# victorvg17/Towards-Interpretable-Reinforcement-Learning-Using-Attention-Augmented-Agents-Replication

Hardware: AMD Instinct MI355X
Metric: learner frames/sec (fwd+bwd, T=20 unroll) at 1/2/4/8 MI355X + % roofline (higher is better)
Workload: dtype fp32; 1 GPU; C2 (BASELINE.json configs[1]): B=32 per GPU x T=20 unroll, 84x84, 4 heads, fp32; global_batch=32, seq_len=20, frame=84x84, heads=4, parallelism=dp1

## Files before the change

### towards-interpretable-reinforcement-learning-using-attention-augmented-agents-replication_amd/csrc/gemm.h

```cpp
#pragma once
#include <type_traits>
#include "common.h"

namespace aaa {

template <typename T, int R, int BK, bool KC>
struct Tile {
  static constexpr int PAD = (!KC && sizeof(T) == 2) ? 32 : 16 / (int)sizeof(T);
  static constexpr int LD = KC ? (BK + PAD) : (R + PAD);
  static constexpr int ELEMS = (KC ? R : BK) * LD;
  __device__ static __forceinline__ int off(int r, int k) { return KC ? r * LD + k : k * LD + r; }
};

template <typename G, typename T, int R, int BK, int NT>
struct LdRows {
  static constexpr bool KC = true;
  static constexpr int VG = 16 / (int)sizeof(G);
  static constexpr int CPR = BK / VG;
  static constexpr int NCH = R * CPR;
  static constexpr int PER = (NCH + NT - 1) / NT;
  struct Params { const G* src; int ld; int nrows; };
  const G* rowp[PER];
  int kc[PER], lr[PER];
  bool ok[PER], act[PER];
// ... 196 lines not shown
  using Regs = u32x4[PER];
  __device__ __forceinline__ LdIm2colT(const Params& p, int row0) : g(p.g), src(p.src) {
#pragma unroll
    for (int c = 0; c < PER; ++c) {
      int ch = threadIdx.x + c * NT;
      act[c] = ch < NCH;
      kr[c] = ch / CPK;
      rc[c] = (ch % CPK) * VG;
      constexpr int NE = VEC ? 1 : 4;
#pragma unroll
      for (int e = 0; e < NE; ++e) {
        int kp = row0 + rc[c] + e;
        rok[c][e] = act[c] && kp < p.nrows;
        int kq = rok[c][e] ? kp : 0;
        int tap = (int)g.dCin.div(kq);
        ci[c][e] = kq - tap * g.Cin;
        ky[c][e] = (int)g.dKW.div(tap);
        kx[c][e] = tap - ky[c][e] * g.KW;
      }
    }
  }
  __device__ __forceinline__ void fetch(int k0, int kend, Regs& buf) const {
    const int hw = g.Hout * g.Wout;
#pragma unroll
    for (int c = 0; c < PER; ++c) {
      u32x4 v = u32x4{0, 0, 0, 0};
      int m = k0 + kr[c];
      if (act[c] && m < kend) {
        int f = (int)g.dHW.div(m), pix = m - f * hw;
        int oy = (int)g.dWout.div(pix), ox = pix - oy * g.Wout;
        const G* fb = src + (size_t)f * g.Hin * g.Win * g.cs + g.coff;
        if constexpr (VEC) {
          int iy, ix;
          if (rok[c][0] && conv_src(g, oy, ox, ky[c][0], kx[c][0], iy, ix))
            v = *reinterpret_cast<const u32x4*>(fb + (size_t)(iy * g.Win + ix) * g.cs + ci[c][0]);
        } else {
          static_assert(sizeof(G) == 4, "scalar im2col path expects fp32 global data");
          float tmp[4] = {0.f, 0.f, 0.f, 0.f};
#pragma unroll
          for (int e = 0; e < 4; ++e) {
            int iy, ix;
            if (rok[c][e] && conv_src(g, oy, ox, ky[c][e], kx[c][e], iy, ix))
              tmp[e] = (float)fb[(size_t)(iy * g.Win + ix) * g.cs + ci[c][e]];
          }
          v = __builtin_bit_cast(u32x4, tmp);
        }
      }
      buf[c] = v;
    }
  }
  __device__ __forceinline__ void commit(T* lds, const Regs& buf) const {
#pragma unroll
    for (int c = 0; c < PER; ++c)
      if (NCH % NT == 0 || act[c]) lds_store_chunk<G, T>(lds + Tile<T, R, BK, false>::off(rc[c], kr[c]), buf[c]);
  }
};

template <typename TL>
__device__ __forceinline__ void frag_f32(const float* t, int r, int k, float (&a)[8]) {
  if constexpr (TL::KC_) {
    const f32x4* p = reinterpret_cast<const f32x4*>(t + r * TL::LD + k);
    f32x4 x = p[0], y = p[1];
    a[0] = x[0]; a[1] = x[1]; a[2] = x[2]; a[3] = x[3];
    a[4] = y[0]; a[5] = y[1]; a[6] = y[2]; a[7] = y[3];
  } else {
#pragma unroll
    for (int kk = 0; kk < 8; ++kk) a[kk] = t[(k + kk) * TL::LD + r];
  }
}

typedef short s16x4 __attribute__((ext_vector_type(4)));
typedef __attribute__((address_space(3))) s16x4 lds_s16x4;

template <typename TL>
__device__ __forceinline__ bf16x8 frag_bf16(const __bf16* t, int r, int k) {
  if constexpr (TL::KC_) {
    return *reinterpret_cast<const bf16x8*>(t + r * TL::LD + k);
  } else {
    const int li = (int)(threadIdx.x & 15), q = li >> 2, p = li & 3;
    const __bf16* a0 = t + (k + q) * TL::LD + (r - li) + 4 * p;
    const s16x4 lo = __builtin_amdgcn_ds_read_tr16_b64_v4i16((lds_s16x4*)(const_cast<__bf16*>(a0)));
    const s16x4 hi = __builtin_amdgcn_ds_read_tr16_b64_v4i16((lds_s16x4*)(const_cast<__bf16*>(a0 + 4 * TL::LD)));
    typedef short s16x8 __attribute__((ext_vector_type(8)));
    const s16x8 v = {lo[0], lo[1], lo[2], lo[3], hi[0], hi[1], hi[2], hi[3]};
    return __builtin_bit_cast(bf16x8, v);
  }
}

struct TileMap {
  int remap;
  FastDiv ny, nxy;
};
__device__ __forceinline__ void tile_of(const TileMap& m, int& ti, int& tj, int& tz) {
  if (!m.remap) { ti = blockIdx.y; tj = blockIdx.x; tz = blockIdx.z; return; }
  const int ny = (int)m.ny.d, nxy = (int)m.nxy.d, n = nxy * gridDim.z;
  const int b = (blockIdx.z * ny + blockIdx.y) * gridDim.x + blockIdx.x;
  const int q = n >> 3, r = n & 7, x = b & 7;
  const int t = (x < r ? x * (q + 1) : r * (q + 1) + (x - r) * q) + (b >> 3);
  tz = (int)m.nxy.div((uint32_t)t);
  const int u = t - tz * nxy;
  tj = (int)m.ny.div((uint32_t)u);
  ti = u - tj * ny;
}
inline int xcd_remap_enabled() {
#ifdef AAA_ABLATION
  const char* e = getenv("AAA_XCD_REMAP");
  return e ? atoi(e) != 0 : 1;
#else
  return 1;
#endif
}
inline TileMap tile_map(dim3 grid) {
  TileMap m;
  m.remap = xcd_remap_enabled();
  m.ny = FastDiv(grid.y);
  m.nxy = FastDiv(grid.x * grid.y);
  return m;
}

template <typename T, int R, int BK, bool KC>
struct TileK : Tile<T, R, BK, KC> { static constexpr bool KC_ = KC; };

template <typename T, int BI_, int BJ_, int BK_, int WI_, int WJ_, int WK_ = 1>
struct GemmCfg {
  using type = T;
  static constexpr int BI = BI_, BJ = BJ_, BK = BK_, WI = WI_, WJ = WJ_, WK = WK_;
  static constexpr int NT = WI * WJ * WK * 64;
};

template <class C, class = void> struct split3_of : std::false_type {};
template <class C> struct split3_of<C, std::enable_if_t<C::SPLIT3>> : std::true_type {};
template <int BI_, int BJ_, int BK_, int WI_, int WJ_, int WK_ = 1>
struct GemmCfgS3 : GemmCfg<float, BI_, BJ_, BK_, WI_, WJ_, WK_> {
  static constexpr bool SPLIT3 = true;
};
template <class C, class = void> struct split6_of : std::false_type {};
template <class C> struct split6_of<C, std::enable_if_t<C::SPLIT6>> : std::true_type {};
template <int BI_, int BJ_, int BK_, int WI_, int WJ_, int WK_ = 1>
struct GemmCfgS6 : GemmCfg<float, BI_, BJ_, BK_, WI_, WJ_, WK_> {
  static constexpr bool SPLIT3 = true, SPLIT6 = true;
};
template <class C, class = void> struct split6l_of : std::false_type {};
template <class C> struct split6l_of<C, std::enable_if_t<C::SPLIT6L>> : std::true_type {};
template <int BI_, int BJ_, int BK_, int WI_, int WJ_, int FD_ = 1>
struct GemmCfgS6L : GemmCfg<float, BI_, BJ_, BK_, WI_, WJ_, 1> {
  static constexpr bool SPLIT3 = true, SPLIT6 = true, SPLIT6L = true;
  static constexpr int FD = FD_;
};
template <int BI_, int BJ_, int BK_, int WI_, int WJ_, int FD_ = 2>
struct GemmCfgS3L : GemmCfg<float, BI_, BJ_, BK_, WI_, WJ_, 1> {
  static constexpr bool SPLIT3 = true, SPLIT6L = true, TWO_PARTS = true;
  static constexpr int FD = FD_;
};
template <class C, class = void> struct two_parts_of : std::false_type {};
template <class C> struct two_parts_of<C, std::enable_if_t<C::TWO_PARTS>> : std::true_type {};
__device__ __forceinline__ void lds_store_split2(__bf16* dst, int plane, const u32x4& raw) {
  const f32x4 f = __builtin_bit_cast(f32x4, raw);
  bf16x4 hi, lo;
#pragma unroll
  for (int e = 0; e < 4; ++e) {
    hi[e] = (__bf16)f[e];
    lo[e] = (__bf16)(f[e] - (float)hi[e]);
  }
  *reinterpret_cast<bf16x4*>(dst) = hi;
  *reinterpret_cast<bf16x4*>(dst + plane) = lo;
}
template <class C, class = void> struct bexact_of : std::false_type {};
template <class C> struct bexact_of<C, std::enable_if_t<C::BEXACT>> : std::true_type {};
template <int BI_, int BJ_, int BK_, int WI_, int WJ_, int WK_ = 1>
struct GemmCfgS6BX : GemmCfgS6<BI_, BJ_, BK_, WI_, WJ_, WK_> {
  static constexpr bool BEXACT = true;
};
template <int BI_, int BJ_, int BK_, int WI_, int WJ_, int FD_ = 1>
struct GemmCfgS6LBX : GemmCfgS6L<BI_, BJ_, BK_, WI_, WJ_, FD_> {
  static constexpr bool BEXACT = true;
};
__device__ __forceinline__ bf16x8 to_bf16x8(const float (&x)[8]) {
  bf16x8 r;
#pragma unroll
  for (int e = 0; e < 8; ++e) r[e] = (__bf16)x[e];
  return r;
}
__device__ __forceinline__ void split3_bf16(const float (&x)[8], bf16x8& hi, bf16x8& mid, bf16x8& lo) {
#pragma unroll
  for (int e = 0; e < 8; ++e) {
    hi[e] = (__bf16)x[e];
    const float r = x[e] - (float)hi[e];
    mid[e] = (__bf16)r;
    lo[e] = (__bf16)(r - (float)mid[e]);
  }
}

__device__ __forceinline__ void lds_store_split3(__bf16* dst, int plane, const u32x4& raw) {
  const f32x4 f = __builtin_bit_cast(f32x4, raw);
  bf16x4 hi, mid, lo;
#pragma unroll
  for (int e = 0; e < 4; ++e) {
    hi[e] = (__bf16)f[e];
    const float r = f[e] - (float)hi[e];
    mid[e] = (__bf16)r;
    lo[e] = (__bf16)(r - (float)mid[e]);
  }
  *reinterpret_cast<bf16x4*>(dst) = hi;
  *reinterpret_cast<bf16x4*>(dst + plane) = mid;
  *reinterpret_cast<bf16x4*>(dst + 2 * plane) = lo;
}

__device__ __forceinline__ void split_bf16(const float (&x)[8], bf16x8& hi, bf16x8& lo) {
#pragma unroll
  for (int e = 0; e < 8; ++e) {
    hi[e] = (__bf16)x[e];
    lo[e] = (__bf16)(x[e] - (float)hi[e]);
  }
}

template <class C, class TA, class TB, int MI, int MJ>
__device__ __forceinline__ void gemm_mma_tile(const typename C::type* Ac, const typename C::type* Bc,
                                              f32x16 (&acc)[MI][MJ], int wi, int wj, int wk, int r32, int h) {
  using T = typename C::type;
  constexpr int BK = C::BK, WK = C::WK, WTI = C::BI / C::WI, WTJ = C::BJ / C::WJ;
#pragma unroll
  for (int s2 = 0; s2 < BK / 16 / WK; ++s2) {
    const int kofs = 16 * (s2 * WK + wk) + 8 * h;
    if constexpr (is_f32<T>::value) {
      float af[MI][8], bfr[MJ][8];
#pragma unroll
      for (int a = 0; a < MI; ++a) frag_f32<TA>(Ac, wi * WTI + a * 32 + r32, kofs, af[a]);
#pragma unroll
      for (int b = 0; b < MJ; ++b) frag_f32<TB>(Bc, wj * WTJ + b * 32 + r32, kofs, bfr[b]);
      if constexpr (split6_of<C>::value) {
        bf16x8 ah[MI], am[MI], al[MI], bh[MJ], bm[MJ], bl[MJ];
#pragma unroll
        for (int a = 0; a < MI; ++a) split3_bf16(af[a], ah[a], am[a], al[a]);
#pragma unroll
        for (int b = 0; b < MJ; ++b) split3_bf16(bfr[b], bh[b], bm[b], bl[b]);
#pragma unroll
        for (int a = 0; a < MI; ++a)
#pragma unroll
          for (int b = 0; b < MJ; ++b) {
            acc[a][b] = __builtin_amdgcn_mfma_f32_32x32x16_bf16(al[a], bh[b], acc[a][b], 0, 0, 0);
            acc[a][b] = __builtin_amdgcn_mfma_f32_32x32x16_bf16(ah[a], bl[b], acc[a][b], 0, 0, 0);
            acc[a][b] = __builtin_amdgcn_mfma_f32_32x32x16_bf16(am[a], bm[b], acc[a][b], 0, 0, 0);
            acc[a][b] = __builtin_amdgcn_mfma_f32_32x32x16_bf16(am[a], bh[b], acc[a][b], 0, 0, 0);
            acc[a][b] = __builtin_amdgcn_mfma_f32_32x32x16_bf16(ah[a], bm[b], acc[a][b], 0, 0, 0);
            acc[a][b] = __builtin_amdgcn_mfma_f32_32x32x16_bf16(ah[a], bh[b], acc[a][b], 0, 0, 0);
          }
      } else if constexpr (split3_of<C>::value) {
        bf16x8 ah[MI], al[MI], bh[MJ], bl[MJ];
#pragma unroll
        for (int a = 0; a < MI; ++a) split_bf16(af[a], ah[a], al[a]);
#pragma unroll
        for (int b = 0; b < MJ; ++b) split_bf16(bfr[b], bh[b], bl[b]);
#pragma unroll
        for (int a = 0; a < MI; ++a)
#pragma unroll
          for (int b = 0; b < MJ; ++b) {
            acc[a][b] = __builtin_amdgcn_mfma_f32_32x32x16_bf16(al[a], bh[b], acc[a][b], 0, 0, 0);
            acc[a][b] = __builtin_amdgcn_mfma_f32_32x32x16_bf16(ah[a], bl[b], acc[a][b], 0, 0, 0);
            acc[a][b] = __builtin_amdgcn_mfma_f32_32x32x16_bf16(ah[a], bh[b], acc[a][b], 0, 0, 0);
          }
      } else {
#pragma unroll
        for (int kk = 0; kk < 8; ++kk)
#pragma unroll
          for (int a = 0; a < MI; ++a)
#pragma unroll
            for (int b = 0; b < MJ; ++b)
              acc[a][b] = __builtin_amdgcn_mfma_f32_32x32x2f32(af[a][kk], bfr[b][kk], acc[a][b], 0, 0, 0);
      }
    } else {
      bf16x8 af[MI], bfr[MJ];
#pragma unroll
      for (int a = 0; a < MI; ++a) af[a] = frag_bf16<TA>(Ac, wi * WTI + a * 32 + r32, kofs);
#pragma unroll
      for (int b = 0; b < MJ; ++b) bfr[b] = frag_bf16<TB>(Bc, wj * WTJ + b * 32 + r32, kofs);
#pragma unroll
      for (int a = 0; a < MI; ++a)
#pragma unroll
        for (int b = 0; b < MJ; ++b)
          acc[a][b] = __builtin_amdgcn_mfma_f32_32x32x16_bf16(af[a], bfr[b], acc[a][b], 0, 0, 0);
    }
  }
}

template <class C, class LA, class LB, class EP>
__global__ void __launch_bounds__(C::NT)
gemm_kernel(typename LA::Params pa, typename LB::Params pb, EP ep, int K, int kchunk, TileMap tm) {
  using T = typename C::type;
  constexpr int BI = C::BI, BJ = C::BJ, BK = C::BK, WI = C::WI, WJ = C::WJ, WK = C::WK;
  constexpr int WTI = BI / WI, WTJ = BJ / WJ, MI = WTI / 32, MJ = WTJ / 32;
  static_assert(MI >= 1 && MJ >= 1 && BK % (16 * WK) == 0, "tile shape");
  using TA = TileK<T, BI, BK, LA::KC>;
  using TB = TileK<T, BJ, BK, LB::KC>;
  __shared__ __attribute__((aligned(16))) T smem[2 * (TA::ELEMS + TB::ELEMS)];
  T* const As0 = smem;
  T* const As1 = smem + TA::ELEMS;
  T* const Bs0 = smem + 2 * TA::ELEMS;
  T* const Bs1 = Bs0 + TB::ELEMS;

  int ti, tj, tz;
  tile_of(tm, ti, tj, tz);
  const int i0 = ti * BI, j0 = tj * BJ;
  const int kb = tz * kchunk;
  const int ke = min(K, kb + kchunk);
  if (kb >= ke) return;

  LA la(pa, i0);
  LB lb(pb, j0);
  const int lane = threadIdx.x & 63, wave = threadIdx.x >> 6;
  const int wk = wave / (WI * WJ), wr = wave - wk * (WI * WJ);
  const int wi = wr / WJ, wj = wr - (wr / WJ) * WJ;
  const int r32 = lane & 31, h = lane >> 5;

  f32x16 acc[MI][MJ];
#pragma unroll
  for (int a = 0; a < MI; ++a)
#pragma unroll
    for (int b = 0; b < MJ; ++b)
#pragma unroll
      for (int e = 0; e < 16; ++e) acc[a][b][e] = 0.f;

  const int nk = (ke - kb + BK - 1) / BK;
  typename LA::Regs ra;
  typename LB::Regs rb;
  la.fetch(kb, ke, ra);
  lb.fetch(kb, ke, rb);
  la.commit(As0, ra);
  lb.commit(Bs0, rb);
  __syncthreads();

  for (int kt = 0; kt < nk; ++kt) {
    const bool odd = kt & 1;
    const T* Ac = odd ? As1 : As0;
    const T* Bc = odd ? Bs1 : Bs0;
    const bool more = kt + 1 < nk;
    if (more) {
      la.fetch(kb + (kt + 1) * BK, ke, ra);
      lb.fetch(kb + (kt + 1) * BK, ke, rb);
    }
    gemm_mma_tile<C, TA, TB, MI, MJ>(Ac, Bc, acc, wi, wj, wk, r32, h);
    if (more) {
      la.commit(odd ? As0 : As1, ra);
      lb.commit(odd ? Bs0 : Bs1, rb);
    }
    __syncthreads();
  }

  if constexpr (WK > 1) {
    constexpr int RED = (WK - 1) * WI * WJ * MI * MJ * 16 * 64;
    static_assert(RED * sizeof(float) <= sizeof(smem), "split-K reduction does not fit in LDS");
    float* red = reinterpret_cast<float*>(smem);
    if (wk > 0) {
#pragma unroll
      for (int a = 0; a < MI; ++a)
#pragma unroll
        for (int b = 0; b < MJ; ++b)
#pragma unroll
          for (int e = 0; e < 16; ++e)
            red[((((wk - 1) * WI * WJ + wr) * MI * MJ + a * MJ + b) * 16 + e) * 64 + lane] = acc[a][b][e];
    }
    __syncthreads();
    if (wk > 0) return;
#pragma unroll
    for (int w = 1; w < WK; ++w)
#pragma unroll
      for (int a = 0; a < MI; ++a)
#pragma unroll
        for (int b = 0; b < MJ; ++b)
#pragma unroll
          for (int e = 0; e < 16; ++e)
            acc[a][b][e] += red[((((w - 1) * WI * WJ + wr) * MI * MJ + a * MJ + b) * 16 + e) * 64 + lane];
  }
#pragma unroll
  for (int a = 0; a < MI; ++a)
#pragma unroll
    for (int b = 0; b < MJ; ++b)
#pragma unroll
      for (int g = 0; g < 4; ++g) {
        const int i = i0 + wi * WTI + a * 32 + 8 * g + 4 * h;
        const int j = j0 + wj * WTJ + b * 32 + r32;
        ep(i, j, acc[a][b][4 * g], acc[a][b][4 * g + 1], acc[a][b][4 * g + 2], acc[a][b][4 * g + 3]);
      }
}

template <class C, class LA, class LB, class EP>
__global__ void __launch_bounds__(C::NT)
gemm_kernel_s6l(typename LA::Params pa, typename LB::Params pb, EP ep, int K, int kchunk, TileMap tm) {
  constexpr int BI = C::BI, BJ = C::BJ, BK = C::BK, WI = C::WI, WJ = C::WJ;
  constexpr int WTI = BI / WI, WTJ = BJ / WJ, MI = WTI / 32, MJ = WTJ / 32;
  static_assert(C::WK == 1 && MI >= 1 && MJ >= 1 && BK % 16 == 0, "tile shape");
  using TA = TileK<__bf16, BI, BK, LA::KC>;
  using TB = TileK<__bf16, BJ, BK, LB::KC>;
  constexpr bool TWO = two_parts_of<C>::value;
  constexpr int NPT = TWO ? 2 : 3;
  constexpr int PA = TA::ELEMS, PB = TB::ELEMS, STG = NPT * (PA + PB);
  constexpr bool BX = bexact_of<C>::value;
  static_assert(!(TWO && BX), "exact B: three-part configs only");
  __shared__ __attribute__((aligned(16))) __bf16 smem[2 * STG];

  int ti, tj, tz;
  tile_of(tm, ti, tj, tz);
  const int i0 = ti * BI, j0 = tj * BJ;
  const int kb = tz * kchunk;
  const int ke = min(K, kb + kchunk);
  if (kb >= ke) return;

  LA la(pa, i0);
  LB lb(pb, j0);
  auto commit_a = [&](__bf16* dst, const typename LA::Regs& r) {
    if constexpr (TWO) la.commit2(dst, PA, r);
    else la.commit3(dst, PA, r);
  };
  auto commit_b = [&](__bf16* dst, const typename LB::Regs& r) {
    if constexpr (BX) lb.commit1(dst, r);
    else if constexpr (TWO) lb.commit2(dst, PB, r);
    else lb.commit3(dst, PB, r);
  };
  const int lane = threadIdx.x & 63, wave = threadIdx.x >> 6;
  const int wi = wave / WJ, wj = wave - (wave / WJ) * WJ;
  const int r32 = lane & 31, h = lane >> 5;

  f32x16 acc[MI][MJ];
#pragma unroll
  for (int a = 0; a < MI; ++a)
#pragma unroll
    for (int b = 0; b < MJ; ++b)
#pragma unroll
      for (int e = 0; e < 16; ++e) acc[a][b][e] = 0.f;

  const int nk = (ke - kb + BK - 1) / BK;
  constexpr int FD = C::FD;
  typename LA::Regs ra[FD];
  typename LB::Regs rb[FD];
  la.fetch(kb, ke, ra[0]);
  lb.fetch(kb, ke, rb[0]);
  if constexpr (FD == 2) {
    if (nk > 1) {
      la.fetch(kb + BK, ke, ra[1]);
      lb.fetch(kb + BK, ke, rb[1]);
    }
  }
  commit_a(smem, ra[0]);
  commit_b(smem + NPT * PA, rb[0]);
  __syncthreads();

  auto step = [&](int kt, auto E) {
    constexpr int e = decltype(E)::value;
    const __bf16* cur = smem + e * STG;
    __bf16* nxt = smem + (e ^ 1) * STG;
    const bool more = kt + 1 < nk;
    if constexpr (FD == 2) {
      la.fetch(kb + (kt + 2) * BK, ke, ra[e]);
      lb.fetch(kb + (kt + 2) * BK, ke, rb[e]);
    } else if (more) {
      la.fetch(kb + (kt + 1) * BK, ke, ra[0]);
      lb.fetch(kb + (kt + 1) * BK, ke, rb[0]);
    }
#pragma unroll
    for (int s2 = 0; s2 < BK / 16; ++s2) {
      const int kofs = 16 * s2 + 8 * h;
      bf16x8 af[MI][3], bfr[MJ][3];
#pragma unroll
      for (int a = 0; a < MI; ++a)
#pragma unroll
        for (int p = 0; p < NPT; ++p) af[a][p] = frag_bf16<TA>(cur + p * PA, wi * WTI + a * 32 + r32, kofs);
#pragma unroll
      for (int b = 0; b < MJ; ++b)
#pragma unroll
        for (int p = 0; p < (BX ? 1 : NPT); ++p)
          bfr[b][p] = frag_bf16<TB>(cur + NPT * PA + p * PB, wj * WTJ + b * 32 + r32, kofs);
      if constexpr (TWO) {
#pragma unroll
        for (int a = 0; a < MI; ++a)
#pragma unroll
          for (int b = 0; b < MJ; ++b) {
            acc[a][b] = __builtin_amdgcn_mfma_f32_32x32x16_bf16(af[a][1], bfr[b][0], acc[a][b], 0, 0, 0);
            acc[a][b] = __builtin_amdgcn_mfma_f32_32x32x16_bf16(af[a][0], bfr[b][1], acc[a][b], 0, 0, 0);
            acc[a][b] = __builtin_amdgcn_mfma_f32_32x32x16_bf16(af[a][0], bfr[b][0], acc[a][b], 0, 0, 0);
          }
      } else
#pragma unroll
      for (int a = 0; a < MI; ++a)
#pragma unroll
        for (int b = 0; b < MJ; ++b) {
          acc[a][b] = __builtin_amdgcn_mfma_f32_32x32x16_bf16(af[a][2], bfr[b][0], acc[a][b], 0, 0, 0);
          if constexpr (!BX) {
            acc[a][b] = __builtin_amdgcn_mfma_f32_32x32x16_bf16(af[a][0], bfr[b][2], acc[a][b], 0, 0, 0);
            acc[a][b] = __builtin_amdgcn_mfma_f32_32x32x16_bf16(af[a][1], bfr[b][1], acc[a][b], 0, 0, 0);
          }
          acc[a][b] = __builtin_amdgcn_mfma_f32_32x32x16_bf16(af[a][1], bfr[b][0], acc[a][b], 0, 0, 0);
          if constexpr (!BX) acc[a][b] = __builtin_amdgcn_mfma_f32_32x32x16_bf16(af[a][0], bfr[b][1], acc[a][b], 0, 0, 0);
          acc[a][b] = __builtin_amdgcn_mfma_f32_32x32x16_bf16(af[a][0], bfr[b][0], acc[a][b], 0, 0, 0);
        }
    }
    if (more) {
      constexpr int rs1 = FD == 2 ? (e ^ 1) : 0;
      commit_a(nxt, ra[rs1]);
      commit_b(nxt + NPT * PA, rb[rs1]);
    }
    __syncthreads();
  };
  for (int kt = 0; kt < nk; kt += 2) {
    step(kt, std::integral_constant<int, 0>{});
    if (kt + 1 < nk) step(kt + 1, std::integral_constant<int, 1>{});
  }
#pragma unroll
  for (int a = 0; a < MI; ++a)
#pragma unroll
    for (int b = 0; b < MJ; ++b)
#pragma unroll
      for (int g = 0; g < 4; ++g) {
        const int i = i0 + wi * WTI + a * 32 + 8 * g + 4 * h;
        const int j = j0 + wj * WTJ + b * 32 + r32;
        ep(i, j, acc[a][b][4 * g], acc[a][b][4 * g + 1], acc[a][b][4 * g + 2], acc[a][b][4 * g + 3]);
      }
}

template <class C, class LA, class LB, class EP>
inline hipError_t launch_gemm(const typename LA::Params& pa, const typename LB::Params& pb, const EP& ep,
                              int Mi, int Nj, int K, int nsplit, hipStream_t st) {
  if (Mi <= 0 || Nj <= 0 || K <= 0) return hipSuccess;
  if (nsplit < 1) nsplit = 1;
  int kchunk = (K + nsplit - 1) / nsplit;
  kchunk = (kchunk + C::BK - 1) / C::BK * C::BK;
  nsplit = (K + kchunk - 1) / kchunk;
  dim3 grid((Nj + C::BJ - 1) / C::BJ, (Mi + C::BI - 1) / C::BI, nsplit);
  if constexpr (split6l_of<C>::value)
    hipLaunchKernelGGL((gemm_kernel_s6l<C, LA, LB, EP>), grid, dim3(C::NT), 0, st, pa, pb, ep, K, kchunk,
                       tile_map(grid));
  else
    hipLaunchKernelGGL((gemm_kernel<C, LA, LB, EP>), grid, dim3(C::NT), 0, st, pa, pb, ep, K, kchunk,
                       tile_map(grid));
  return hipGetLastError();
}

}
```

### towards-interpretable-reinforcement-learning-using-attention-augmented-agents-replication_amd/csrc/rt_backward.hip

```cpp
#include "rt.h"

namespace aaa {


template <typename T>
static int conv2_dgrad(const Layout& L, const char* pk, const T* dy2, T* dy1, int frames, float* gbias,
                       hipStream_t s) {
  {
    constexpr int CKd = std::is_same<T, float>::value ? 32 : 64;
    const int Ha = (L.H1 + 1) / 2, Wa = (L.W1 + 1) / 2;
    auto halo4 = [&](auto cfg, auto nbuf) -> int {
      using HC = decltype(cfg);
      EpiStoreParity4<T> ep(dy1, frames * Ha * Wa, Ha, Wa, L.H1, L.W1, gbias);
      const HaloParams hp{pk + L.k_WdT2, 256, 128, dy2, 64, 0, 64, (uint32_t)((size_t)frames * L.P * 64 * L.esz),
                          L.h, L.w, frames, 0, Ha, Wa};
      HIPCHK((launch_halo<HC, EpiStoreParity4<T>, 2, decltype(nbuf)::value>(hp, ep, s)));
      return AAA_OK;
    };
    using NB3 = std::integral_constant<int, 3>;
    auto fits = [&](int fr, int bj, int hmax) {
      return fr * Ha * Wa <= bj && fr * (L.h + 2) * (L.w + 2) + 1 <= hmax && Ha <= L.h && Wa <= L.w;
    };
    const int fr = ab_int("AAA_DGRAD2_FR", std::is_same<T, float>::value ? 1 : 2);
    if (ab_int("AAA_DGRAD2_HALO", 1)) {
// ... 34 lines not shown
                                             : classes(GemmCfg<T, 32, 128, BKd, 1, 4>{});
  }
  if constexpr (!std::is_same<T, float>::value) return fail(AAA_E_ARG, "AAA_CONV2_DGRAD_RING=0 needs fp32");
  using C3 = Cfg32For<T>;
  using LA = LdRowsB<T, T, C3::BI, C3::BK, C3::NT>;
  using LB = LdIm2colB<float, T, C3::BJ, C3::BK, C3::NT>;
  for (int cls = 0; cls < 4; ++cls) {
    const int py = cls >> 1, px = cls & 1;
    const int Ha = (L.H1 - py + 1) / 2, Wa = (L.W1 - px + 1) / 2;
    if (Ha <= 0 || Wa <= 0) continue;
    const int rows = frames * Ha * Wa;
    typename LA::Params pa{(const T*)(pk + L.k_WdT2) + (size_t)cls * 32 * 256, 256, 32};
    typename LB::Params pb{(const float*)dy2, ConvGeo{64, 64, 0, L.h, L.w, Ha, Wa, 2, 1, 0, 0}.prep(), rows,
                           (uint32_t)((size_t)frames * L.P * 64 * 4)};
    EpiStoreParity ep{(float*)dy1, 32, rows, Ha, Wa, L.H1, L.W1, py, px, FastDiv((uint32_t)(Ha * Wa)),
                      FastDiv((uint32_t)Wa)};
    HIPCHK((launch_gemm<C3, LA, LB>(pa, pb, ep, 32, rows, 256, 1, s)));
  }
  return AAA_OK;
}

template <typename T>
static int conv2_wgrad(const Layout& L, const T* dy2, const T* y1, int frames, float* gW, hipStream_t s) {
  using C = CfgFor<T>;
  using LA = LdRowsTB<T, T, C::BI, C::BK, C::NT>;
  using LB = LdIm2colTB<T, T, C::BJ, C::BK, C::NT>;
  const int rows = frames * L.P;
  if constexpr (!std::is_same<T, float>::value) {
    const int pipe = ab_int("AAA_CONV2_WGRAD_PIPE", 1);
    if (rows % 32 == 0 && pipe) {
      using CW = GemmCfg<T, 64, 256, 32, 1, 4>;
      using PA = GRowsT<T, CW::BI, CW::BK, CW::NT>;
      using PB = GIm2colT<T, CW::BJ, CW::BK, CW::NT>;
      typename PA::Params pa{dy2, 64, 64, rows};
      typename PB::Params pb{y1, ConvGeo{32, 32, 0, L.H1, L.W1, L.h, L.w, 4, 2, 2, 0}.prep(), 512,
                             (uint32_t)((size_t)frames * L.P1 * 32 * L.esz)};
      EpiAtomicD ep{{gW, 512, 64, 512}};
      const int ns = std::max(1, std::min(ab_int("AAA_CONV2_WGRAD_WGS", 256) / 2, rows / (8 * CW::BK)));
      if (pipe == 2) HIPCHK((launch_pipe_ra<CW, PA, PB, EpiAtomicD, 4>(pa, pb, ep, 64, 512, rows, ns, s)));
      else HIPCHK((launch_pipe<CW, PA, PB, EpiAtomicD, 4, 2>(pa, pb, ep, 64, 512, rows, ns, s)));
      return AAA_OK;
    }
  }
  typename LA::Params pa{dy2, 64, 64, rows};
  typename LB::Params pb{y1, ConvGeo{32, 32, 0, L.H1, L.W1, L.h, L.w, 4, 2, 2, 0}.prep(), 512,
                         (uint32_t)((size_t)frames * L.P1 * 32 * L.esz)};
  EpiStore<true> ep{gW, 512, 64, 512};
  const int tiles = cdiv(64, C::BI) * cdiv(512, C::BJ);
  if constexpr (std::is_same<T, float>::value) {
    if (f32_split6()) {
      auto s6l = [&](auto cfg, int ns) -> int {
        using CW = decltype(cfg);
        using LA6 = LdRowsTB<T, T, CW::BI, CW::BK, CW::NT>;
        using LB6 = LdIm2colTB<T, T, CW::BJ, CW::BK, CW::NT>;
        typename LA6::Params pa6{dy2, 64, 64, rows};
        typename LB6::Params pb6{y1, ConvGeo{32, 32, 0, L.H1, L.W1, L.h, L.w, 4, 2, 2, 0}.prep(), 512,
                                 (uint32_t)((size_t)frames * L.P1 * 32 * L.esz)};
        HIPCHK((launch_gemm<CW, LA6, LB6>(pa6, pb6, ep, 64, 512, rows, std::max(1, std::min(ns, rows / 128)), s)));
        return AAA_OK;
      };
#ifdef AAA_ABLATION
      const int c2s = ab_int("AAA_CONV2_WGRAD_S6L", 0);
      if (c2s == 1) return s6l(GemmCfgS6L<64, 256, 16, 1, 4, 2>{}, 256);
      if (c2s == 2) return s6l(GemmCfgS6L<64, 256, 16, 2, 4, 2>{}, 128);
      if (c2s == 3) return s6l(GemmCfgS6L<64, 128, 16, 1, 2, 2>{}, 256);
#else
      (void)s6l;
#endif
      HIPCHK((launch_gemm<typename S6Of<C>::type, LA, LB>(pa, pb, ep, 64, 512, rows, wgrad_splits(tiles, rows, C::BK), s)));
      return AAA_OK;
    }
  }
  HIPCHK((launch_gemm<C, LA, LB>(pa, pb, ep, 64, 512, rows, wgrad_splits(tiles, rows, C::BK), s)));
  return AAA_OK;
}

template <typename T>
static int conv1_wgrad(const Layout& L, const T* dy1, const T* xp, int frames, float* gW, hipStream_t s) {
  const int rows1 = frames * L.P1;
  auto run = [&](auto cfg) -> int {
    using C3 = decltype(cfg);
    using LA = LdRowsTB<T, T, C3::BI, C3::BK, C3::NT>;
    using LB = LdIm2colTB<T, T, C3::BJ, C3::BK, C3::NT>;
    typename LA::Params pa{dy1, 32, 32, rows1};
    typename LB::Params pb{xp, ConvGeo{4, 4, 0, L.H + 2, L.W + 2, L.H1, L.W1, 8, 4, 0, 0}.prep(), 256,
                           (uint32_t)((size_t)frames * (L.H + 2) * (L.W + 2) * 4 * L.esz)};
    EpiStore<true> ep{gW, 256, 32, 256};
    const int tiles = cdiv(32, C3::BI) * cdiv(256, C3::BJ);
    if constexpr (std::is_same<T, float>::value) {
      if (f32_split6()) {
        HIPCHK((launch_gemm<typename S6Of<C3>::type, LA, LB>(pa, pb, ep, 32, 256, rows1,
                                                            wgrad_splits(tiles, rows1, C3::BK), s)));
        return AAA_OK;
      }
    }
    HIPCHK((launch_gemm<C3, LA, LB>(pa, pb, ep, 32, 256, rows1, wgrad_splits(tiles, rows1, C3::BK), s)));
    return AAA_OK;
  };
  if constexpr (!std::is_same<T, float>::value) {
    const int pipe = ab_int("AAA_CONV1_WGRAD_PIPE", 1);
    if (rows1 % 64 == 0 && pipe) {
      using CW = GemmCfg<T, 32, 256, 64, 1, 4>;
      using PA = GRowsT<T, CW::BI, CW::BK, CW::NT>;
      using PB = GIm2colT<T, CW::BJ, CW::BK, CW::NT>;
      typename PA::Params pa{dy1, 32, 32, rows1};
      typename PB::Params pb{xp, ConvGeo{4, 4, 0, L.H + 2, L.W + 2, L.H1, L.W1, 8, 4, 0, 0}.prep(), 256,
                             (uint32_t)((size_t)frames * (L.H + 2) * (L.W + 2) * 4 * L.esz)};
      EpiAtomicD ep{{gW, 256, 32, 256}};
      const int ns = std::max(1, std::min(ab_int("AAA_CONV1_WGRAD_WGS", 256), rows1 / (8 * CW::BK)));
      if (pipe == 2) HIPCHK((launch_pipe_ra<CW, PA, PB, EpiAtomicD, 4>(pa, pb, ep, 32, 256, rows1, ns, s)));
      else HIPCHK((launch_pipe<CW, PA, PB, EpiAtomicD, 4, 2>(pa, pb, ep, 32, 256, rows1, ns, s)));
      return AAA_OK;
    }
  }
  if constexpr (std::is_same<T, float>::value) {
    const int c1s = f32_split6() ? ab_int("AAA_CONV1_WGRAD_S6L", 1) : 0;
    auto s6l = [&](auto cfg, int ns) -> int {
      using CW = decltype(cfg);
      using LA6 = LdRowsTB<T, T, CW::BI, CW::BK, CW::NT>;
      using LB6 = LdIm2colTB<T, T, CW::BJ, CW::BK, CW::NT>;
      typename LA6::Params pa6{dy1, 32, 32, rows1};
      typename LB6::Params pb6{xp, ConvGeo{4, 4, 0, L.H + 2, L.W + 2, L.H1, L.W1, 8, 4, 0, 0}.prep(), 256,
                               (uint32_t)((size_t)frames * (L.H + 2) * (L.W + 2) * 4 * L.esz)};
      EpiStore<true> ep6{gW, 256, 32, 256};
      HIPCHK((launch_gemm<CW, LA6, LB6>(pa6, pb6, ep6, 32, 256, rows1, std::max(1, std::min(ns, rows1 / 128)), s)));
      return AAA_OK;
    };
    if (c1s == 1)
      return L.fu8 && ab_int("AAA_CONV1_BEXACT", 1) ? s6l(GemmCfgS6LBX<32, 256, 16, 1, 4, 2>{}, 512)
                                                     : s6l(GemmCfgS6L<32, 256, 16, 1, 4, 2>{}, 512);
#ifdef AAA_ABLATION
    if (c1s == 2) return s6l(GemmCfgS6L<32, 256, 16, 1, 4, 2>{}, 256);
    if (c1s == 3) return s6l(GemmCfgS6L<32, 128, 16, 1, 2, 2>{}, 512);
#endif
  }
  if (ab_int("AAA_CONV1_WGRAD_TILE", 0) == 1) return run(GemmCfg<T, 32, 256, Cfg32For<T>::BK, 1, 4>{});
  return run(Cfg32For<T>{});
}

template <typename T>
int lstm_wgrad(const T* dz, const T* xh, int rows, int h, int w, float* gW, hipStream_t s, bool aux) {
  const uint32_t xh_bytes = (uint32_t)((size_t)rows * 192 * sizeof(T));
  auto wgrad_lstm = [&](auto cfg) -> int {
    using CW = decltype(cfg);
    using LA = LdRowsTB<T, T, CW::BI, CW::BK, CW::NT>;
    using LB = LdIm2colTB<T, T, CW::BJ, CW::BK, CW::NT>;
    typename LA::Params pa{dz, 512, 512, rows};
    typename LB::Params pb{xh, ConvGeo{192, 192, 0, h, w, h, w, 3, 1, 1, 0}.prep(),
                           1728, xh_bytes};
    EpiStore<true> ep{gW, 1728, 512, 1728};
    const int tiles = cdiv(512, CW::BI) * cdiv(1728, CW::BJ);
    const int per_cu = split6l_of<CW>::value ? device_cus() : 512;
    const int ns = std::max(1, std::min(ab_int("AAA_WGRAD_SPLIT", std::max(1, per_cu / tiles)), rows / CW::BK));
    TimerScope tim(AAA_TIMER_CORE_WGRAD, s, 2.0 * 512 * 1728 * rows,
                   strf("register-staged %dx%d BK%d%s, %d-way split-K atomics [kernel: gemm_kernel+%d, %d, %d, +LdIm2colTB]",
                        CW::BI, CW::BJ, CW::BK, split6_of<CW>::value ? " (fp32 as bf16x6 split products)" : "", ns,
                        CW::BI, CW::BJ, CW::BK));
    HIPCHK((launch_gemm<CW, LA, LB>(pa, pb, ep, 512, 1728, rows, ns, s)));
    return AAA_OK;
  };
  auto wgrad_lstm_pipe = [&](auto cfg, auto nbuf, auto ilv) -> int {
    using CW = decltype(cfg);
    constexpr int NB = decltype(nbuf)::value, IL = decltype(ilv)::value;
    using LA = GRowsT<T, CW::BI, CW::BK, CW::NT>;
    using LB = GIm2colT<T, CW::BJ, CW::BK, CW::NT>;
    typename LA::Params pa{dz, 512, 512, rows};
    typename LB::Params pb{xh, ConvGeo{192, 192, 0, h, w, h, w, 3, 1, 1, 0}.prep(),
                           1728, xh_bytes};
    EpiAtomicD ep{{gW, 1728, 512, 1728}};
    const int tiles = cdiv(512, CW::BI) * cdiv(1728, CW::BJ);
    TimerScope tim(AAA_TIMER_CORE_WGRAD, s, 2.0 * 512 * 1728 * rows, strf("LDS-DMA ring %dx%d BK%d, %d-deep [kernel: gemm_pipe_kernel+GIm2colT]", CW::BI, CW::BJ, CW::BK, NB));
    const int wgs = ab_int("AAA_WGRAD_WGS", 256);
    const int ns = std::max(1, std::min(wgs / tiles, rows / (8 * CW::BK)));
    HIPCHK((launch_pipe<CW, LA, LB, EpiAtomicD, NB, IL>(pa, pb, ep, 512, 1728, rows, ns, s)));
    return AAA_OK;
  };
  auto wgrad_lstm_ra = [&](auto cfg, auto nbuf) -> int {
    using CW = decltype(cfg);
    constexpr int NB = decltype(nbuf)::value;
    using LA = GRowsT<T, CW::BI, CW::BK, CW::NT>;
    using LB = GIm2colT<T, CW::BJ, CW::BK, CW::NT>;
    typename LA::Params pa{dz, 512, 512, rows};
    typename LB::Params pb{xh, ConvGeo{192, 192, 0, h, w, h, w, 3, 1, 1, 0}.prep(), 1728, xh_bytes};
    EpiAtomicD ep{{gW, 1728, 512, 1728}};
    const int tiles = cdiv(512, CW::BI) * cdiv(1728, CW::BJ);
    TimerScope tim(AAA_TIMER_CORE_WGRAD, s, 2.0 * 512 * 1728 * rows,
                   strf("LDS-DMA read-ahead ring %dx%d BK%d, %d-deep [kernel: gemm_pipe_ra_kernel+GIm2colT]", CW::BI, CW::BJ, CW::BK, NB));
    const int wgs = ab_int("AAA_WGRAD_WGS", 256);
    const int ns = std::max(1, std::min(wgs / tiles, rows / (8 * CW::BK)));
    HIPCHK((launch_pipe_ra<CW, LA, LB, EpiAtomicD, NB>(pa, pb, ep, 512, 1728, rows, ns, s)));
    return AAA_OK;
  };
  constexpr int WBK = std::is_same<T, float>::value ? 32 : 64;
  const int wpipe = rows % WBK == 0 ? env_int("AAA_WGRAD_PIPE", std::is_same<T, float>::value || aux ? 0 : 9) : 0;
  if (wpipe) {
    using I0 = std::integral_constant<int, 0>;
    using I2 = std::integral_constant<int, 2>;
    using I3 = std::integral_constant<int, 3>;
    int rc;
    switch (wpipe) {
      case 2: rc = wgrad_lstm_pipe(GemmCfg<T, 256, 128, WBK, 2, 2>{}, I2{}, I0{}); break;
      case 3:
        if constexpr (std::is_same<T, float>::value) rc = wgrad_lstm_pipe(GemmCfg<T, 256, 128, WBK, 2, 2>{}, I2{}, I0{});
        else rc = wgrad_lstm_pipe(GemmCfg<T, 256, 256, WBK, 2, 4>{}, I2{}, I0{});
        break;
      case 4: rc = wgrad_lstm_pipe(GemmCfg<T, 128, 256, WBK, 2, 2>{}, I2{}, I0{}); break;
      case 5: rc = wgrad_lstm_pipe(GemmCfg<T, 256, 128, WBK, 2, 2>{}, I3{}, I0{}); break;
      case 6:
      case 7:
        if constexpr (std::is_same<T, float>::value)
          rc = wgrad_lstm_pipe(GemmCfg<T, 128, 128, WBK, 2, 2>{}, I3{}, I2{});
        else if (wpipe == 6)
          rc = wgrad_lstm_pipe(GemmCfg<T, 256, 256, 32, 2, 4>{}, std::integral_constant<int, 4>{}, I2{});
        else
          rc = wgrad_lstm_pipe(GemmCfg<T, 256, 256, 32, 2, 4>{}, I3{}, I2{});
        break;
      case 8:
        if constexpr (std::is_same<T, float>::value)
          rc = wgrad_lstm_pipe(GemmCfg<T, 128, 128, WBK, 2, 2>{}, I3{}, I2{});
        else
          rc = wgrad_lstm_pipe(GemmCfg<T, 256, 256, 32, 2, 2>{}, std::integral_constant<int, 4>{}, I2{});
        break;
      case 9:
        if constexpr (std::is_same<T, float>::value)
          rc = wgrad_lstm_pipe(GemmCfg<T, 128, 128, WBK, 2, 2>{}, I3{}, I2{});
        else
          rc = wgrad_lstm_ra(GemmCfg<T, 256, 256, 32, 2, 4>{}, std::integral_constant<int, 4>{});
        break;
      default: rc = wgrad_lstm_pipe(GemmCfg<T, 128, 128, WBK, 2, 2>{}, I2{}, I0{}); break;
    }
    if (rc) return rc;
  } else if (std::is_same<T, float>::value && f32_split6()) {
    auto s6 = [&](auto cfg) {
      using CS6 = std::conditional_t<std::is_same<T, float>::value, decltype(cfg), CfgWFor<T>>;
      return wgrad_lstm(CS6{});
    };
#ifdef AAA_ABLATION
    const int tile6 = ab_int("AAA_WGRAD_S6_TILE", 6);
    const int rc = tile6 == 1   ? s6(GemmCfgS6<128, 256, 32, 2, 2>{})
                   : tile6 == 2 ? s6(GemmCfgS6<256, 128, 32, 2, 2>{})
                   : tile6 == 3 ? s6(GemmCfgS6<256, 256, 32, 2, 4>{})
                   : tile6 == 4 ? s6(GemmCfgS6L<256, 256, 16, 2, 4>{})
                   : tile6 == 5 ? s6(GemmCfgS6L<256, 128, 16, 2, 2>{})
                   : tile6 == 6 ? s6(GemmCfgS6L<256, 256, 16, 2, 4, 2>{})
                   : tile6 == 7 ? s6(GemmCfgS6L<256, 192, 16, 4, 2, 2>{})
                                : s6(GemmCfgS6<128, 128, 32, 2, 2>{});
#else
    const int rc = s6(GemmCfgS6L<256, 256, 16, 2, 4, 2>{});
#endif
    if (rc) return rc;
  } else {
    const int wide = ab_int("AAA_AUX_WIDE", aux ? 0 : 1);
#ifdef AAA_ABLATION
    const int rc = !wide ? wgrad_lstm(CfgFor<T>{})
                   : ab_int("AAA_WGRAD_TILE", 0) == 1 ? wgrad_lstm(GemmCfg<T, 128, 192, 32, 2, 2>{})
                                                       : wgrad_lstm(CfgWFor<T>{});
#else
    const int rc = !wide ? wgrad_lstm(CfgFor<T>{}) : wgrad_lstm(CfgWFor<T>{});
#endif
    if (rc) return rc;
  }
  return AAA_OK;
}

template <typename T>
static int conv1_wgrad_frames(const Layout& L, const T* dy1, const void* frames, int n, T* xpbuf, float* gW,
                              hipStream_t s) {
  const size_t fb = (size_t)L.H * L.W * 3 * (L.fu8 ? 1 : 4);
  for (int s0 = 0; s0 < n; s0 += L.xpc) {
    const int m = std::min(L.xpc, n - s0);
    const char* fr = (const char*)frames + (size_t)s0 * fb;
    if (L.fu8) HIPCHK((frames_rgbx<T, uint8_t>(m, L.H, L.W, (const uint8_t*)fr, xpbuf, s)));
    else HIPCHK((frames_rgbx<T, float>(m, L.H, L.W, (const float*)fr, xpbuf, s)));
    const int rc = conv1_wgrad<T>(L, dy1 + (size_t)s0 * L.P1 * 32, xpbuf, m, gW, s);
    if (rc) return rc;
  }
  return AAA_OK;
}

template <typename T>
int vision_bwd(const Layout& L, const char* pk, const T* dy2, const T* y1, T* xp, T* dy1, int F,
                      float* gW2, float* gW1, float* gb1, hipStream_t s, const void* frames) {
  const size_t fb = (size_t)L.H * L.W * 3 * (L.fu8 ? 1 : 4);
  for (int f0 = 0; f0 < F; f0 += L.fchunk) {
    const int n = std::min(L.fchunk, F - f0);
    const T* d2 = dy2 + (size_t)f0 * L.P * 64;
    T* d1 = dy1 + (size_t)f0 * L.P1 * 32;
    int rc = conv2_wgrad<T>(L, d2, y1 + (size_t)f0 * L.P1 * 32, n, gW2, s);
    if (!rc) rc = conv2_dgrad<T>(L, pk, d2, d1, n, gb1, s);
    if (!rc && frames) rc = conv1_wgrad_frames<T>(L, d1, (const char*)frames + (size_t)f0 * fb, n, xp, gW1, s);
    else if (!rc) rc = conv1_wgrad<T>(L, d1, xp + (size_t)f0 * (L.H + 2) * (L.W + 2) * 4, n, gW1, s);
    if (rc) return rc;
  }
  return AAA_OK;
}

template <typename T>
static bool vbwd_on(const Layout& L, int F) {
  if constexpr (!std::is_same<T, __bf16>::value) {
    (void)L; (void)F;
    return false;
  } else {
    return L.fu8 && vbwd_fits(L.H, L.W, L.H1, L.W1, L.h, L.w) && env_int("AAA_VIS_FRAMES", 1) &&
           env_int("AAA_VIS_BWD_FRAMES", 1) && F >= env_int("AAA_VBWD_MINF", 0) * device_cus() &&
           (size_t)vbwd_groups(F, device_cus()) * kVbPart * 4 <= (size_t)F * L.P1 * 32 * L.esz;
  }
// ... 701 lines not shown
```

Baseline: 236,600 frames/s.

## Interleave LDS commits among MFMAs and pair the K loop in LSTM wgrad

Adds a GemmCfgS6LK variant of the split-6 register-staged GEMM. It runs the K loop in unconditional pairs and, using sched_group_barrier hints, places the LDS commits of the next stage between the bf16x6 MFMAs instead of after them. It always prefetches the second tile, so it relies on the fetch bounds-checking past ke. This is the default path for the LSTM weight-gradient GEMM when the config qualifies. An ablation-only ping-pong kernel, with the waves in two halves alternating between compute and staging, is also added but not selected by default.

```diff
diff --git a/towards-interpretable-reinforcement-learning-using-attention-augmented-agents-replication_amd/csrc/gemm.h b/towards-interpretable-reinforcement-learning-using-attention-augmented-agents-replication_amd/csrc/gemm.h
--- a/towards-interpretable-reinforcement-learning-using-attention-augmented-agents-replication_amd/csrc/gemm.h
+++ b/towards-interpretable-reinforcement-learning-using-attention-augmented-agents-replication_amd/csrc/gemm.h
@@ -372,6 +372,15 @@
   static constexpr bool SPLIT3 = true, SPLIT6L = true, TWO_PARTS = true;
   static constexpr int FD = FD_;
 };
+template <int BI_, int BJ_, int BK_, int WI_, int WJ_, int FD_ = 2, int CI_ = 1>
+struct GemmCfgS6LK : GemmCfgS6L<BI_, BJ_, BK_, WI_, WJ_, FD_> {
+  static constexpr bool KPAIRS = true;
+  static constexpr bool COMMIT_ILV = CI_ != 0;
+};
+template <class C, class = void> struct kpairs_of : std::false_type {};
+template <class C> struct kpairs_of<C, std::enable_if_t<C::KPAIRS>> : std::true_type {};
+template <class C, class = void> struct commit_ilv_of : std::false_type {};
+template <class C> struct commit_ilv_of<C, std::enable_if_t<C::KPAIRS>> : std::integral_constant<bool, C::COMMIT_ILV> {};
 template <class C, class = void> struct two_parts_of : std::false_type {};
 template <class C> struct two_parts_of<C, std::enable_if_t<C::TWO_PARTS>> : std::true_type {};
 __device__ __forceinline__ void lds_store_split2(__bf16* dst, int plane, const u32x4& raw) {
@@ -655,7 +664,7 @@
   la.fetch(kb, ke, ra[0]);
   lb.fetch(kb, ke, rb[0]);
   if constexpr (FD == 2) {
-    if (nk > 1) {
+    if (nk > 1 || commit_ilv_of<C>::value) {
       la.fetch(kb + BK, ke, ra[1]);
       lb.fetch(kb + BK, ke, rb[1]);
     }
@@ -676,6 +685,7 @@
       la.fetch(kb + (kt + 1) * BK, ke, ra[0]);
       lb.fetch(kb + (kt + 1) * BK, ke, rb[0]);
     }
+    constexpr int rs1 = FD == 2 ? (e ^ 1) : 0;
 #pragma unroll
     for (int s2 = 0; s2 < BK / 16; ++s2) {
       const int kofs = 16 * s2 + 8 * h;
@@ -713,13 +723,28 @@
           acc[a][b] = __builtin_amdgcn_mfma_f32_32x32x16_bf16(af[a][0], bfr[b][0], acc[a][b], 0, 0, 0);
         }
     }
-    if (more) {
-      constexpr int rs1 = FD == 2 ? (e ^ 1) : 0;
+    if constexpr (commit_ilv_of<C>::value) {
       commit_a(nxt, ra[rs1]);
       commit_b(nxt + NPT * PA, rb[rs1]);
+      __builtin_amdgcn_sched_group_barrier(0x8, 12, 0);
+#pragma unroll
+      for (int i = 0; i < 6 * MI * MJ * (BK / 16) - 12; ++i) {
+        __builtin_amdgcn_sched_group_barrier(0x8, 1, 0);
+        __builtin_amdgcn_sched_group_barrier(0x2, 3, 0);
+      }
+    } else if (more) {
+      commit_a(nxt, ra[rs1]);
+      commit_b(nxt + NPT * PA, rb[rs1]);
     }
     __syncthreads();
   };
+  if constexpr (kpairs_of<C>::value) {
+    for (int kt = 0; kt + 1 < nk; kt += 2) {
+      step(kt, std::integral_constant<int, 0>{});
+      step(kt + 1, std::integral_constant<int, 1>{});
+    }
+    if (nk & 1) step(nk - 1, std::integral_constant<int, 0>{});
+  } else
   for (int kt = 0; kt < nk; kt += 2) {
     step(kt, std::integral_constant<int, 0>{});
     if (kt + 1 < nk) step(kt + 1, std::integral_constant<int, 1>{});
@@ -734,6 +759,175 @@
         const int j = j0 + wj * WTJ + b * 32 + r32;
         ep(i, j, acc[a][b][4 * g], acc[a][b][4 * g + 1], acc[a][b][4 * g + 2], acc[a][b][4 * g + 3]);
       }
+}
+
+template <class C, class = void> struct s6p_of : std::false_type {};
+template <class C>
+struct s6p_of<C, std::enable_if_t<C::SPLIT6L && C::SPLIT6 && C::FD == 2 && C::WI * C::WJ == 8>>
+    : std::integral_constant<bool, !bexact_of<C>::value> {};
+
+template <class C, class LA, class LB, class EP, int V = 5>
+__global__ void __launch_bounds__(C::NT)
+gemm_kernel_s6p(typename LA::Params pa, typename LB::Params pb, EP ep, int K, int kchunk, TileMap tm) {
+  constexpr int BI = C::BI, BJ = C::BJ, BK = C::BK, WI = C::WI, WJ = C::WJ;
+  constexpr int WTI = BI / WI, WTJ = BJ / WJ, MI = WTI / 32, MJ = WTJ / 32;
+  static_assert(C::WK == 1 && MI >= 1 && MJ >= 1 && BK % 16 == 0, "tile shape");
+  static_assert(C::FD == 2 && !two_parts_of<C>::value && !bexact_of<C>::value, "three-part FD 2 configs");
+  static_assert(WI * WJ == 8, "two halves of four waves: one wave of each half per SIMD");
+  using TA = TileK<__bf16, BI, BK, LA::KC>;
+  using TB = TileK<__bf16, BJ, BK, LB::KC>;
+  constexpr int PA = TA::ELEMS, PB = TB::ELEMS, STG = 3 * (PA + PB);
+  __shared__ __attribute__((aligned(16))) __bf16 smem[2 * STG];
+
+  int ti, tj, tz;
+  tile_of(tm, ti, tj, tz);
+  const int i0 = ti * BI, j0 = tj * BJ;
+  const int kb = tz * kchunk;
+  const int ke = min(K, kb + kchunk);
+  if (kb >= ke) return;
+
+  LA la(pa, i0);
+  LB lb(pb, j0);
+  const int lane = threadIdx.x & 63, wave = __builtin_amdgcn_readfirstlane(threadIdx.x >> 6);
+  const int wi = wave / WJ, wj = wave - (wave / WJ) * WJ;
+  const int r32 = lane & 31, h = lane >> 5;
+  const bool half1 = wave >= 4;
+  if constexpr (V & 1) {
+    if (half1) __builtin_amdgcn_s_setprio(1);
+  }
+
+  f32x16 acc[MI][MJ];
+#pragma unroll
+  for (int a = 0; a < MI; ++a)
+#pragma unroll
+    for (int b = 0; b < MJ; ++b)
+#pragma unroll
+      for (int e = 0; e < 16; ++e) acc[a][b][e] = 0.f;
+
+  const int nk = (ke - kb + BK - 1) / BK;
+  typename LA::Regs ra[2];
+  typename LB::Regs rb[2];
+  la.fetch(kb, ke, ra[0]);
+  lb.fetch(kb, ke, rb[0]);
+  la.fetch(kb + BK, ke, ra[1]);
+  lb.fetch(kb + BK, ke, rb[1]);
+  la.commit3(smem, PA, ra[0]);
+  lb.commit3(smem + 3 * PA, PB, rb[0]);
+  if constexpr (!(V & 4)) {
+    la.fetch(kb + 2 * BK, ke, ra[0]);
+    lb.fetch(kb + 2 * BK, ke, rb[0]);
+  }
+  __syncthreads();
+
+  auto mma = [&](const __bf16* cur) {
+    auto fa = [&](int a, int p, int kofs) { return frag_bf16<TA>(cur + p * PA, wi * WTI + a * 32 + r32, kofs); };
+    auto fb = [&](int b, int p, int kofs) {
+      return frag_bf16<TB>(cur + 3 * PA + p * PB, wj * WTJ + b * 32 + r32, kofs);
+    };
+    auto six = [&](f32x16& d, const bf16x8 (&x)[3], const bf16x8 (&y)[3]) {
+      d = __builtin_amdgcn_mfma_f32_32x32x16_bf16(x[2], y[0], d, 0, 0, 0);
+      d = __builtin_amdgcn_mfma_f32_32x32x16_bf16(x[0], y[2], d, 0, 0, 0);
+      d = __builtin_amdgcn_mfma_f32_32x32x16_bf16(x[1], y[1], d, 0, 0, 0);
+      d = __builtin_amdgcn_mfma_f32_32x32x16_bf16(x[1], y[0], d, 0, 0, 0);
+      d = __builtin_amdgcn_mfma_f32_32x32x16_bf16(x[0], y[1], d, 0, 0, 0);
+      d = __builtin_amdgcn_mfma_f32_32x32x16_bf16(x[0], y[0], d, 0, 0, 0);
+    };
+#pragma unroll
+    for (int s2 = 0; s2 < BK / 16; ++s2) {
+      const int kofs = 16 * s2 + 8 * h;
+      bf16x8 bfr[MJ][3];
+      if constexpr (V & 2) {
+        bf16x8 af[2][3];
+#pragma unroll
+        for (int p = 0; p < 3; ++p) af[0][p] = fa(0, p, kofs);
+#pragma unroll
+        for (int b = 0; b < MJ; ++b)
+#pragma unroll
+          for (int p = 0; p < 3; ++p) bfr[b][p] = fb(b, p, kofs);
+#pragma unroll
+        for (int a = 0; a < MI; ++a) {
+          if (a + 1 < MI) {
+#pragma unroll
+            for (int p = 0; p < 3; ++p) af[(a + 1) & 1][p] = fa(a + 1, p, kofs);
+          }
+          __builtin_amdgcn_sched_barrier(0);
+#pragma unroll
+          for (int b = 0; b < MJ; ++b) six(acc[a][b], af[a & 1], bfr[b]);
+          __builtin_amdgcn_sched_barrier(0);
+        }
+      } else {
+        bf16x8 af[MI][3];
+#pragma unroll
+        for (int a = 0; a < MI; ++a)
+#pragma unroll
+          for (int p = 0; p < 3; ++p) af[a][p] = fa(a, p, kofs);
+#pragma unroll
+        for (int b = 0; b < MJ; ++b)
+#pragma unroll
+          for (int p = 0; p < 3; ++p) bfr[b][p] = fb(b, p, kofs);
+#pragma unroll
+        for (int a = 0; a < MI; ++a)
+#pragma unroll
+          for (int b = 0; b < MJ; ++b) six(acc[a][b], af[a], bfr[b]);
+      }
+    }
+  };
+  auto stage = [&](int kt, auto E) {
+    constexpr int e = decltype(E)::value;
+    __bf16* nxt = smem + (e ^ 1) * STG;
+    if constexpr (V & 4) {
+      la.fetch(kb + (kt + 2) * BK, ke, ra[e]);
+      lb.fetch(kb + (kt + 2) * BK, ke, rb[e]);
+    }
+    if (kt + 1 < nk) {
+      la.commit3(nxt, PA, ra[e ^ 1]);
+      lb.commit3(nxt + 3 * PA, PB, rb[e ^ 1]);
+    }
+    if constexpr (!(V & 4)) {
+      la.fetch(kb + (kt + 3) * BK, ke, ra[e ^ 1]);
+      lb.fetch(kb + (kt + 3) * BK, ke, rb[e ^ 1]);
+    }
+  };
+  if (half1) {
+    stage(0, std::integral_constant<int, 0>{});
+    __syncthreads();
+  }
+  auto step = [&](int kt, auto E) {
+    constexpr int e = decltype(E)::value;
+    mma(smem + e * STG);
+    __syncthreads();
+    if (!half1) stage(kt, E);
+    else if (kt + 1 < nk) stage(kt + 1, std::integral_constant<int, e ^ 1>{});
+    if (!half1 || kt + 1 < nk) __syncthreads();
+  };
+  for (int kt = 0; kt < nk; kt += 2) {
+    step(kt, std::integral_constant<int, 0>{});
+    if (kt + 1 < nk) step(kt + 1, std::integral_constant<int, 1>{});
+  }
+#pragma unroll
+  for (int a = 0; a < MI; ++a)
+#pragma unroll
+    for (int b = 0; b < MJ; ++b)
+#pragma unroll
+      for (int g = 0; g < 4; ++g) {
+        const int i = i0 + wi * WTI + a * 32 + 8 * g + 4 * h;
+        const int j = j0 + wj * WTJ + b * 32 + r32;
+        ep(i, j, acc[a][b][4 * g], acc[a][b][4 * g + 1], acc[a][b][4 * g + 2], acc[a][b][4 * g + 3]);
+      }
+}
+
+template <class C, class LA, class LB, int V = 5, class EP>
+inline hipError_t launch_gemm_s6p(const typename LA::Params& pa, const typename LB::Params& pb, const EP& ep,
+                                  int Mi, int Nj, int K, int nsplit, hipStream_t st) {
+  if (Mi <= 0 || Nj <= 0 || K <= 0) return hipSuccess;
+  if (nsplit < 1) nsplit = 1;
+  int kchunk = (K + nsplit - 1) / nsplit;
+  kchunk = (kchunk + C::BK - 1) / C::BK * C::BK;
+  nsplit = (K + kchunk - 1) / kchunk;
+  dim3 grid((Nj + C::BJ - 1) / C::BJ, (Mi + C::BI - 1) / C::BI, nsplit);
+  hipLaunchKernelGGL((gemm_kernel_s6p<C, LA, LB, EP, V>), grid, dim3(C::NT), 0, st, pa, pb, ep, K, kchunk,
+                     tile_map(grid));
+  return hipGetLastError();
 }
 
 template <class C, class LA, class LB, class EP>
diff --git a/towards-interpretable-reinforcement-learning-using-attention-augmented-agents-replication_amd/csrc/rt_backward.hip b/towards-interpretable-reinforcement-learning-using-attention-augmented-agents-replication_amd/csrc/rt_backward.hip
--- a/towards-interpretable-reinforcement-learning-using-attention-augmented-agents-replication_amd/csrc/rt_backward.hip
+++ b/towards-interpretable-reinforcement-learning-using-attention-augmented-agents-replication_amd/csrc/rt_backward.hip
@@ -210,6 +210,30 @@
     const int tiles = cdiv(512, CW::BI) * cdiv(1728, CW::BJ);
     const int per_cu = split6l_of<CW>::value ? device_cus() : 512;
     const int ns = std::max(1, std::min(ab_int("AAA_WGRAD_SPLIT", std::max(1, per_cu / tiles)), rows / CW::BK));
+    if constexpr (s6p_of<CW>::value) {
+      int sched = env_int("AAA_WGRAD_S6_PAIRED", 1);
+#ifndef AAA_ABLATION
+      if (sched > 1) sched = 1;
+#endif
+      auto run = [&](auto cfg, const char* what, auto paired) -> int {
+        using CK = decltype(cfg);
+        TimerScope tim(AAA_TIMER_CORE_WGRAD, s, 2.0 * 512 * 1728 * rows,
+                       strf("register-staged %dx%d BK%d (fp32 as bf16x6 split products), %s, %d-way split-K atomics "
+                            "[kernel: %s+LdIm2colTB]", CW::BI, CW::BJ, CW::BK, what, ns,
+                            decltype(paired)::value ? "gemm_kernel_s6p" : "gemm_kernel_s6l+GemmCfgS6LK"));
+        if constexpr (decltype(paired)::value) HIPCHK((launch_gemm_s6p<CK, LA, LB>(pa, pb, ep, 512, 1728, rows, ns, s)));
+        else HIPCHK((launch_gemm<CK, LA, LB>(pa, pb, ep, 512, 1728, rows, ns, s)));
+        return AAA_OK;
+      };
+      if (sched == 1)
+        return run(GemmCfgS6LK<CW::BI, CW::BJ, CW::BK, CW::WI, CW::WJ, 2, 1>{},
+                   "K loop in pairs, commits among the MFMAs", std::false_type{});
+#ifdef AAA_ABLATION
+      if (sched == 2) return run(CW{}, "paired MFMA / commit segments", std::true_type{});
+      if (sched == 3)
+        return run(GemmCfgS6LK<CW::BI, CW::BJ, CW::BK, CW::WI, CW::WJ, 2, 0>{}, "K loop in pairs", std::false_type{});
+#endif
+    }
     TimerScope tim(AAA_TIMER_CORE_WGRAD, s, 2.0 * 512 * 1728 * rows,
                    strf("register-staged %dx%d BK%d%s, %d-way split-K atomics [kernel: gemm_kernel+%d, %d, %d, +LdIm2colTB]",
                         CW::BI, CW::BJ, CW::BK, split6_of<CW>::value ? " (fp32 as bf16x6 split products)" : "", ns,
```

Result: faster. 239,600 frames/s (median of 6 runs) (+1.3%).
